# neale/safelife-k2

Measured on AMD Instinct MI355X. Metric: env-steps/sec (whole node) on 64×64 boards, batch 65536; bit-exact vs CPU ref, higher is better.
Workload: dtype u16; 1 GPU; 64x64 proc-gen prune-still, PPO wrapper chain; envs_per_gpu=65536, burnin_steps=400, global_batch=65536, parallelism=dp1 (env shards), obs=none, rng=philox, board_mode=auto, read_board=False

## Files before the change

### include/safelife_hip.h

```cpp
#ifndef SAFELIFE_HIP_H
#define SAFELIFE_HIP_H

#include <stdint.h>

#ifdef __cplusplus
extern "C" {
#endif

#define SL_OK 0
#define SL_EINVAL (-1)
#define SL_EHIP (-2)
#define SL_ETOOBIG (-3)

#define SL_RNG_STREAM 0
#define SL_RNG_PHILOX 1

#define SL_KERNEL_AUTO 0
#define SL_KERNEL_GENERIC 1
#define SL_KERNEL_FAST 2
#define SL_KERNEL_BANDS 3

#define SL_STREAM_ERR_RANGE 1
#define SL_STREAM_ERR_THRESHOLD 2

#define SL_BOARD_AUTO 0
#define SL_BOARD_UINT16 1

#define SL_MAX_EXITS 8
#define SL_BONUS_PERIOD_MAX 16

#define SL_OBS_NONE 0
#define SL_OBS_PACKED 1
#define SL_OBS_CHANNELS 2
#define SL_OBS_CHANNELS_U8 3
#define SL_OBS_CHANNELS_F32 4
#define SL_OBS_CHANNELS_BF16 5

const char *sl_version(void);
const char *sl_build_id(void);
int sl_device_arch(char *buf, int len);

int sl_event_create(void **ev);
int sl_event_destroy(void *ev);
int sl_event_elapsed_ms(void *begin, void *end, float *ms);
int sl_copy16(const void *src, void *dst, int64_t n16, void *stream);


int sl_advance(const uint16_t *in, uint16_t *out, int64_t B, int H, int W,
               const float *spawn_prob, float spawn_prob_scalar, int rng_mode,
               uint64_t seed, uint32_t env0, uint32_t step, uint32_t tensor,
               const double *draws, const int64_t *draw_offsets, void *stream);

int sl_count_eligible(const uint16_t *in, int64_t *counts, int64_t B, int H, int W,
                      void *stream);

int64_t sl_host_advance(const uint16_t *in, uint16_t *out, int64_t H, int64_t W,
                        float spawn_prob, const double *draws, int64_t n_draws);

int sl_exclusive_scan_i64(const int64_t *in, int64_t *out, int64_t n,
                          const int64_t *base, int64_t *total_out, void *stream);


#define SL_MT_PREFIX 21216
#define SL_MT_CTL_WORDS 8
#define SL_MT_POLY_WORDS 640
typedef struct sl_mt19937 {
    int32_t n_chains;
    int32_t rounds;
    int64_t ring_draws;
    double *ring;
    uint32_t *chains;
    uint32_t *prefix;
    uint32_t *polys;
    int64_t *ctl;
    void *ahead_stream;
    void *ev_fill, *ev_ahead;
    int32_t ahead_pending;
    int32_t bit_ring;
    double bits_thr;
} sl_mt19937;

int sl_mt19937_seed(sl_mt19937 *mt, uint32_t seed, int64_t first_draw, void *stream);
int sl_mt19937_fill(const sl_mt19937 *mt, const int64_t *lo, const int64_t *hi, int64_t *err,
                    void *stream);
int sl_mt19937_lookahead(sl_mt19937 *mt, void *ahead_stream);
int sl_mt19937_release(sl_mt19937 *mt);
int sl_mt19937_host_window(uint32_t seed, uint32_t *window624);
int sl_mt19937_host_jump_poly(uint64_t n, uint32_t *poly);
int sl_mt19937_host_jump(const uint32_t *window_in, const uint32_t *poly, uint32_t *window_out);
int sl_mt19937_host_draws(const uint32_t *window, int64_t n, double *out);


int sl_emd_cells(const double *p, const double *q, const int32_t *ys, const int32_t *xs,
                 int64_t n, const double *cost_table, int H, int W,
                 double extra_mass_penalty, double *out);

int sl_side_effect_workspace(int64_t E, int H, int W, int64_t *bytes);
int sl_side_effect_densities(const uint16_t *init_board, const uint16_t *final_board,
                             const int32_t *num_steps_dev, const int32_t *num_steps_host,
                             const float *spawn_prob, int64_t E, int H, int W,
                             int num_samples, int rng_mode, uint64_t seed, uint32_t env0,
                             const double *draws, int64_t *stream_pos, int max_keys,
                             uint16_t *keys, int32_t *n_keys, int32_t *present,
                             double *inaction, double *action, void *workspace,
                             int64_t workspace_bytes, void *stream);
int sl_side_effect_densities_k(const uint16_t *init_board, const uint16_t *final_board,
                               const int32_t *num_steps_dev, const int32_t *num_steps_host,
                               const float *spawn_prob, int64_t E, int H, int W,
                               int num_samples, int rng_mode, uint64_t seed, uint32_t env0,
// ... 181 lines not shown
```

### safelife-k2_amd/csrc/sl_bits.h

```cpp
#pragma once
#include "sl_action.h"


namespace sl {
namespace bits {

typedef uint32_t u32;

__device__ __forceinline__ u32 maj(u32 a, u32 b, u32 c) { return (a & b) | (c & (a | b)); }
__device__ __forceinline__ u32 mux(u32 s, u32 a, u32 b) { return (s & a) | (~s & b); }

template <int CTRL>
__device__ __forceinline__ u32 dpp(u32 v) {
    return (u32)__builtin_amdgcn_mov_dpp((int)v, CTRL, 0xF, 0xF, false);
}
__device__ __forceinline__ u32 lane_m1(u32 v) { return dpp<0x13C>(v); }
__device__ __forceinline__ u32 lane_p1(u32 v) { return dpp<0x134>(v); }
__device__ __forceinline__ u32 lane_x1(u32 v) { return dpp<0xB1>(v); }

struct H3 {
    u32 l0, r1;
};
struct V3 {
    u32 up, dn;
// ... 548 lines not shown
    __device__ int baseline() const { return rec(V, R_BASE); }
    __device__ int exit_count() const { return rec(V, R_EXC); }
    __device__ int exit_y(int e) const {
        return (int)(int16_t)(rec(V, R_EY + (e >> 1)) >> (16 * (e & 1)));
    }
    __device__ int exit_x(int e) const {
        return (int)(int16_t)(rec(V, R_EX + (e >> 1)) >> (16 * (e & 1)));
    }
    __device__ int game_over() const { return go; }
    __device__ int agent_x() const { return ax; }
    __device__ int agent_y() const { return ay; }
    __device__ int prior_len() const { return rec(V, R_PLEN); }
    __device__ int prior_head() const { return rec(V, R_PHEAD); }
    __device__ int prior_x(int k) const { return rec(V, R_PX + k); }
    __device__ int prior_y(int k) const { return rec(V, R_PY + k); }
    __device__ int side_effect() const { return rec(V, R_SIDE); }
    __device__ double bonus(int) const { return bval; }
};


__device__ __forceinline__ SpawnCtx spawn_ctx(const StepArgs &a, int64_t b, int spawn_bits) {
    SpawnCtx sc;
    sc.gid = a.env0 + (uint32_t)b;
    sc.step = a.step;
    sc.seed = a.seed;
    set_spawn_prob(sc, __int_as_float(spawn_bits));
    return sc;
}

template <int MODE>
__device__ __forceinline__ StreamSrc stream_src(const StepArgs &a, int64_t *scratch, int64_t B,
                                                int64_t b, int64_t &pos_b, int64_t &pos_g) {
    StreamSrc src{a.draws, a.n_draws, nullptr, a.draw_mask, a.draw_bits};
    pos_b = 0;
    pos_g = 0;
    if (MODE == SPAWN_STREAM) {
        const Scratch w = scratch_of(scratch, B);
        src.err = w.err;
        pos_b = w.offsets[2 * b];
        pos_g = w.offsets[2 * b + 1];
    }
    return src;
}

__device__ __forceinline__ RecFields rec_fields(const StepArgs &a, u32 V, int go, int ax, int ay) {
    RecFields fl{V, go, ax, ay, 0.0};
    if (a.bonus_period > 0)
        fl.bval = a.bonus_table[bonus_dist(fl.ax, fl.ay, fl.prior_x(fl.prior_head()),
                                           fl.prior_y(fl.prior_head()), fl.prior_len(),
                                           a.bonus_period, a.bonus_len)];
    return fl;
}

struct ScoreTotals {
    int points, score, possible, side;
};
__device__ __forceinline__ ScoreTotals score_totals(int pts, int scr, int pos, int side) {
    const int s1 = wave_total((pts + 192) | ((scr + 64) << 16));
    const int s2 = wave_total(pos | (side << 16));
    return ScoreTotals{(s1 & 0xFFFF) - 192 * 64, ((s1 >> 16) & 0xFFFF) - 64 * 64, s2 & 0xFFFF,
                       (s2 >> 16) & 0xFFFF};
}

struct Words2 {
    u32 w[2];
};
__device__ __forceinline__ Words2 recolour_exits(u32 P[32], bool can) {
    Words2 d9;
#pragma unroll
    for (int w = 0; w < 2; w++) {
        const u32 o9 = PL(P, 9, w);
        PL(P, 9, w) = can ? (o9 | PL(P, 8, w)) : (o9 & ~PL(P, 8, w));
        d9.w[w] = o9 ^ PL(P, 9, w);
    }
    return d9;
}

__device__ __forceinline__ void queue_reset(int64_t *scratch, int64_t B, uint32_t step, int64_t b) {
    int64_t *cnt = scratch + 8 * B + 2 + (step & 1);
    const int i = (int)atomicAdd((unsigned long long *)cnt, 1ull);
    reset_list(scratch)[i] = (int32_t)b;
}

}
}
```

### safelife-k2_amd/csrc/sl_bits.hip

```cpp
#include "sl_bits_geo.h"
#include "sl_obs.h"

using namespace sl;
using namespace sl::fast;
using namespace sl::bits;

namespace {

constexpr int kMinWaves = 4;
constexpr int kMinWavesObs = 3;

constexpr int N = 64;

typedef __attribute__((address_space(3))) u32 lds_u32;

__device__ __forceinline__ void dma_board(const uint16_t *__restrict__ src, lds_u32 *buf,
                                          int lane) {
    const char *s = reinterpret_cast<const char *>(src);
#pragma unroll
    for (int k = 0; k < 8; k++) {
        const int q = k * 64 + lane, row = q >> 3, pos = q & 7;
        const int c = (pos - ((row >> 5) << 2)) & 7;
        __builtin_amdgcn_global_load_lds((const void *)(s + row * 128 + c * 16),
                                         (__attribute__((address_space(3))) void *)(buf + k * 256),
// ... 656 lines not shown
struct PlaneSlots {
    static constexpr bool kFixed = K16 == kKeepC3;
    u32 keep;
    u32 store;
    __device__ __forceinline__ u32 keep32() const { return K16 ? K16 * 0x10001u : keep; }
    __device__ __forceinline__ u32 store32() const {
        return kFixed ? (K16 & ~kAgentC3) * 0x10001u : store;
    }
    __device__ __forceinline__ bool kept(int q) const { return (keep32() >> q) & 1u; }
    __device__ __forceinline__ bool stored(int q) const { return (store32() >> q) & 1u; }
    __device__ __forceinline__ u32 agent16() const {
        return kFixed ? kAgentC3 : (keep32() & ~store32()) & 0xFFFFu;
    }
    __device__ __forceinline__ int pos(int q) const {
        if (kFixed) return __builtin_popcount(store32() & ((1u << q) - 1u));
        u32 k = store;
        asm volatile("" : "+s"(k));
        return __builtin_popcount(k & ((1u << q) - 1u));
    }
    __device__ __forceinline__ int stored16() const { return __builtin_popcount(store32() & 0xFFFFu); }
    static __device__ __forceinline__ PlaneSlots of(u32 zero, u32 agent) {
        const u32 k = ~zero & 0xFFFFu;
        return PlaneSlots{k * 0x10001u, (k & ~agent) * 0x10001u};
    }
};
__device__ __forceinline__ void agent_words(int ay, int ax, int lane, u32 aw[2]) {
    const u32 bit = lane == 2 * (ax >> 1) + (ay >> 5) ? 1u << (ay & 31) : 0u;
    aw[0] = (ax & 1) ? 0u : bit;
    aw[1] = (ax & 1) ? bit : 0u;
}
constexpr int kMinWavesPlanes = 5;
constexpr int planes_min_waves(u32 k16, int obs) {
    return (obs == 0 && k16 == kKeepC3) ? kMinWavesPlanes : kMinWaves;
}

template <u32 K16>
__device__ __forceinline__ void dma_planes(const u32 *__restrict__ bp, PlaneSlots<K16> ps,
                                           lds_u32 *buf, int lane) {
    const int groups = (2 * ps.stored16() + 3) >> 2;
    const char *s = reinterpret_cast<const char *>(bp);
#pragma unroll
    for (int g = 0; g < 8; g++)
        if (g < groups)
            __builtin_amdgcn_global_load_lds((const void *)(s + g * 1024 + lane * 16),
                                             (__attribute__((address_space(3))) void *)(buf + g * 256),
                                             16, 0, 2);
}

__device__ __forceinline__ int near_cell_index(int k, int y0, int x0) {
    const int dy = k < 5 ? 0 : (k == 5 ? -1 : k == 6 ? 1 : k == 7 ? -2 : 2);
    const int dx = k >= 5 || k == 0 ? 0 : (k == 1 ? -1 : k == 2 ? 1 : k == 3 ? -2 : 2);
    return ((y0 + dy) & 63) * 64 + ((x0 + dx) & 63);
}
struct NearCells {
    int y0, x0;
    u32 v;
    __device__ __forceinline__ uint32_t operator()(int i) const {
        const int dy = (((i >> 6) - y0 + 32) & 63) - 32, dx = (((i & 63) - x0 + 32) & 63) - 32;
        const int k = dy == 0 ? (dx == 0 ? 0 : dx == -1 ? 1 : dx == 1 ? 2 : dx == -2 ? 3 : 4)
                              : (dy == -1 ? 5 : dy == 1 ? 6 : dy == -2 ? 7 : 8);
        return (u32)__builtin_amdgcn_readlane((int)v, __builtin_amdgcn_readfirstlane(k));
    }
};
template <u32 K16>
__device__ __forceinline__ u32 lds_plane_cell(const lds_u32 *buf, PlaneSlots<K16> ps, int i) {
    const int y = i >> 6, x = i & 63;
    const lds_u32 *q = buf + 2 * (x >> 1) + (y >> 5);
    const u32 r = (u32)(y & 31);
    const int w = 16 * (x & 1);
    u32 v = 0;
#pragma unroll
    for (int p = 0; p < 16; p++) {
        const int pw = ps.pos(p) + (w ? ps.stored16() : 0);
        if (ps.stored(p)) v |= ((q[pw * 64] >> r) & 1u) << p;
    }
    return v;
}

template <u32 K16, int OBS>
__global__ void __launch_bounds__(64, planes_min_waves(K16, OBS))
k_env_step_bits64_planes(StepKArgs ka) {
    __shared__ __attribute__((aligned(16))) u32 stage[N * N / 2];
    uint16_t *const vm = nullptr;
    constexpr bool GRAY = false, W6 = false;
#include "sl_planes64_step.inc"
}

template <u32 K16, int OBS>
__global__ void __launch_bounds__(64, planes_min_waves(K16, OBS))
k_env_planes64_gray(StepKArgs ka) {
    static_assert(OBS <= 1, "channel views load the three colour planes");
    __shared__ __attribute__((aligned(16))) u32 stage[N * N / 2];
    uint16_t *const vm = nullptr;
    constexpr bool GRAY = true, W6 = false;
#include "sl_planes64_step.inc"
}

constexpr int kMinWavesW6 = 6;
constexpr int kStageDwW6 = 1536;
template <u32 K16>
__global__ void __launch_bounds__(64, kMinWavesW6)
k_env_planes64_w6(StepKArgs ka) {
    __shared__ __attribute__((aligned(16))) u32 stage[kStageDwW6];
    uint16_t *const vm = nullptr;
    constexpr int OBS = 0;
    constexpr bool GRAY = true, W6 = true;
#include "sl_planes64_step.inc"
}

template <u32 K16, int ESZ>
__global__ void __launch_bounds__(64, kMinWaves)
k_env_planes64_chan(StepKArgs ka) {
    constexpr int OBS = ESZ == 1 ? 3 : (ESZ == 4 ? 4 : 2);
    __shared__ __attribute__((aligned(16))) u32 stage[N * N / 2];
    __shared__ __attribute__((aligned(16))) uint16_t vmask[sl::obs::kFusedChanCells];
    uint16_t *const vm = vmask;
    constexpr bool GRAY = false, W6 = false;
#include "sl_planes64_step.inc"
}

__global__ void __launch_bounds__(64) k_board_sync64(sl_env_state st, int demote) {
    const int64_t b = blockIdx.x;
    const int lane = threadIdx.x;
    const int pok = __builtin_amdgcn_readfirstlane(st.planes_ok[b]);
    if (!(pok & SL_POK_BOARD_PLANES)) return;
    if (!(pok & SL_POK_BOARD_FULL)) {
        const PlaneSlots<0> ps = PlaneSlots<0>::of(st.board_zero, st.agent_planes);
        const u32 *bp = st.planes + b * 4096 + lane;
        u32 P[32];
#pragma unroll
        for (int q = 0; q < 32; q++) P[q] = ps.stored(q) ? bp[ps.pos(q) * 64] : 0u;
        u32 aw[2];
        agent_words(__builtin_amdgcn_readfirstlane(st.agent_y[b]),
                    __builtin_amdgcn_readfirstlane(st.agent_x[b]), lane, aw);
#pragma unroll
        for (int q = 0; q < 32; q++)
            if ((ps.agent16() >> (q & 15)) & 1u) P[q] = aw[q >> 4];
        transpose32(P);
        u32 *gb = reinterpret_cast<u32 *>(st.board + b * (int64_t)(N * N)) + (lane & 1) * 1024 +
                  (lane >> 1);
#pragma unroll
        for (int y = 0; y < 32; y++) gb[y * 32] = P[y];
    }
    if (lane == 0)
        st.planes_ok[b] = demote ? pok & ~(SL_POK_BOARD_PLANES | SL_POK_BOARD_FULL)
                                 : pok | SL_POK_BOARD_FULL;
}

__global__ void __launch_bounds__(64)
k_stream_prologue64(StepKArgs ka) {
    const sl_env_state &st = ka.st;
    const int64_t b = blockIdx.x;
    const int lane = threadIdx.x;
    const int64_t off = b * (int64_t)(N * N);
    const int lane_off = (lane & 1) * 1024 + (lane >> 1);
    const u32 V = load_record(st, ka.actions, b, lane);
    const Scratch w = scratch_of(ka.fx.scratch, st.B);
    const int spf = rec(V, R_SPF) | (ka.ctp ? 1 : 0);
    SpawnCtx sc{0u, 0u, 0ull, 0.0};
    u32 P[32], ch[2];
    int nb = 0;
    if (spf & 1) {
        load_pairs_nt<32>(reinterpret_cast<const u32 *>(st.board + off) + lane_off, P);
        transpose32(P);
        Geo64<SPAWN_COUNT> gbd{lane, StreamSrc{nullptr, 0, nullptr}, 0, 0};
        rule_planes(P, ch, gbd, sc, 0u);
        nb = wave_total(gbd.count);
    }
    const int pok = (st.planes && st.planes_ok) ? rec(V, R_POK) & kPokGoalsSkip : 0;
    int ng = 0;
    if ((pok & kPokGoalsSkip) != kPokGoalsSkip && (spf & 2)) {
        if (pok & SL_POK_GOALS_MIRROR) {
            const u32 *mg = st.planes + b * 4096 + 2048 + lane;
#pragma unroll
            for (int q = 0; q < 32; q++) P[q] = mg[q * 64];
        } else {
            load_pairs_nt<32>(reinterpret_cast<const u32 *>(st.goals + off) + lane_off, P);
            transpose32(P);
        }
        Geo64<SPAWN_COUNT> ggl{lane, StreamSrc{nullptr, 0, nullptr}, 0, 0};
        rule_planes(P, ch, ggl, sc, 1u);
        ng = wave_total(ggl.count);
    }
    if (lane == 0) {
        w.counts[2 * b] = nb;
        w.counts[2 * b + 1] = ng;
    }
}

__global__ void __launch_bounds__(64)
k_env_reset_list(sl_env_state st, sl_level_pool pool, ResetArgs ra, int64_t *scratch,
                 uint32_t step, sl::obs::ObsArgs oa, uint64_t chpack, uint32_t one,
                 uint16_t *obs_out) {
    __shared__ __attribute__((aligned(16))) uint16_t vmask[sl::obs::kFusedChanCells];
    int64_t *cnt = scratch + 8 * st.B + 2;
    if (blockIdx.x == 0 && threadIdx.x == 0) cnt[(step + 1) & 1] = 0;
    const int32_t *list = reset_list(scratch);
    const int first = list[blockIdx.x];
    const int n = (int)__builtin_amdgcn_readfirstlane((int)cnt[step & 1]);
    for (int i = blockIdx.x; i < n; i += gridDim.x) {
        const int64_t b = __builtin_amdgcn_readfirstlane(i == (int)blockIdx.x ? first : list[i]);
        wave_reset(st, pool, ra, b, threadIdx.x);
        if (obs_out) {
            wait_vm();
            const sl::obs::ChanMap cm{chpack, oa.nch};
            uint8_t *o8 = reinterpret_cast<uint8_t *>(obs_out);
            if (oa.mode == SL_OBS_PACKED)
                sl::obs::obs_packed_wave(st, oa, b, threadIdx.x, obs_out);
            else if (oa.mode == SL_OBS_CHANNELS_U8)
                sl::obs::obs_channels_wave<1>(st, oa, cm, one, b, threadIdx.x, vmask, o8);
            else if (oa.mode == SL_OBS_CHANNELS_F32)
                sl::obs::obs_channels_wave<4>(st, oa, cm, one, b, threadIdx.x, vmask, o8);
            else
                sl::obs::obs_channels_wave<2>(st, oa, cm, one, b, threadIdx.x, vmask, o8);
        }
    }
}

int obs_kind(const FastExtra &fx) {
    if (!fx.obs_out) return 0;
    switch (fx.obs_mode) {
    case SL_OBS_PACKED: return 1;
    case SL_OBS_CHANNELS_U8: return 3;
    case SL_OBS_CHANNELS_F32: return 4;
    default: return 2;
    }
}

template <int MODE>
void launch_bits64(int kind, unsigned grid, const StepKArgs &ka, hipStream_t s) {
    switch (kind) {
    case 0: hipLaunchKernelGGL((k_env_step_bits64<0, MODE>), dim3(grid), dim3(64), 0, s, ka); break;
    case 1: hipLaunchKernelGGL((k_env_step_bits64<1, MODE>), dim3(grid), dim3(64), 0, s, ka); break;
    case 2: hipLaunchKernelGGL((k_env_step_bits64<2, MODE>), dim3(grid), dim3(64), 0, s, ka); break;
    case 3: hipLaunchKernelGGL((k_env_step_bits64<3, MODE>), dim3(grid), dim3(64), 0, s, ka); break;
    default: hipLaunchKernelGGL((k_env_step_bits64<4, MODE>), dim3(grid), dim3(64), 0, s, ka); break;
    }
}

template <u32 K16>
void launch_planes64_chan_k(int esz, unsigned grid, const StepKArgs &ka, hipStream_t s) {
    switch (esz) {
    case 1: hipLaunchKernelGGL((k_env_planes64_chan<K16, 1>), dim3(grid), dim3(64), 0, s, ka); break;
    case 4: hipLaunchKernelGGL((k_env_planes64_chan<K16, 4>), dim3(grid), dim3(64), 0, s, ka); break;
    default: hipLaunchKernelGGL((k_env_planes64_chan<K16, 2>), dim3(grid), dim3(64), 0, s, ka); break;
    }
}

void launch_planes64_chan(u32 keep, int esz, unsigned grid, const StepKArgs &ka, hipStream_t s) {
    if (keep == kKeepC3Fixed) launch_planes64_chan_k<kKeepC3>(esz, grid, ka, s);
    else if (keep == kKeepAll) launch_planes64_chan_k<kKeepAll>(esz, grid, ka, s);
    else launch_planes64_chan_k<0>(esz, grid, ka, s);
}

}

namespace sl {

bool planes64_shape(const sl_env_state &st) {
    return st.H == N && st.W == N && st.planes && st.planes_ok && st.board_planes == st.planes;
}

int sync_board_planes64(const sl_env_state &st, int demote, hipStream_t s) {
    if (!planes64_shape(st) || st.B <= 0) return SL_OK;
    hipLaunchKernelGGL(k_board_sync64, dim3((unsigned)st.B), dim3(64), 0, s, st, demote);
    return hipGetLastError() == hipSuccess ? SL_OK : SL_EHIP;
}

int launch_step_bits(const sl_env_state &st, const StepArgs &a, const FastExtra &fx,
                     const int32_t *actions, int ctp, int ctc, double *reward, uint8_t *done,
                     uint8_t *flags, int32_t *ep_len, int32_t *ep_rew, hipStream_t s,
                     int planes64_waves) {
    if (st.H != N || st.W != N) return SL_ETOOBIG;
    const unsigned grid = (unsigned)st.B;
    const StepKArgs ka{st, a, fx, actions, ctp, ctc, reward, done, flags, ep_len, ep_rew};
    if (fx.obs_out && (fx.obs_vh < 1 || fx.obs_vw < 1 || fx.obs_vh * fx.obs_vw > 4096))
        return SL_EINVAL;
    if (fx.stream) {
        if (stream_counts(fx)) {
            const int rca = launch_env_action(st, actions, ctp, ctc, scratch_of(fx.scratch, st.B).act, s);
            if (rca) return rca;
            hipLaunchKernelGGL(k_stream_prologue64, dim3(grid), dim3(64), 0, s, ka);
            if (hipGetLastError() != hipSuccess) return SL_EHIP;
        }
        const int rc = stream_offsets(st, fx, s);
        if (rc || !stream_steps(fx)) return rc;
        if (fx.ev_begin) (void)hipEventRecord((hipEvent_t)fx.ev_begin, s);
        launch_bits64<SPAWN_STREAM>(obs_kind(fx), grid, ka, s);
    } else {
        if (fx.ev_begin) (void)hipEventRecord((hipEvent_t)fx.ev_begin, s);
        if (fx.plane_mode) {
            u32 keep = ~st.board_zero & 0xFFFFu;
            if (keep == kKeepC3) keep = st.agent_planes == kAgentC3 ? kKeepC3Fixed : 0u;
            const int kind = obs_kind(fx);
            if (kind >= 2) {
                launch_planes64_chan(keep, obs_esz(kind), grid, ka, s);
            } else if (keep == kKeepC3Fixed && st.goals_gray) {
                if (kind)
                    hipLaunchKernelGGL((k_env_planes64_gray<kKeepC3, 1>), dim3(grid), dim3(64), 0, s, ka);
                else if (planes64_waves == 5)
                    hipLaunchKernelGGL((k_env_planes64_gray<kKeepC3, 0>), dim3(grid), dim3(64), 0, s, ka);
                else
                    hipLaunchKernelGGL((k_env_planes64_w6<kKeepC3>), dim3(grid), dim3(64), 0, s, ka);
            } else if (fx.obs_out) {
                if (keep == kKeepC3Fixed)
                    hipLaunchKernelGGL((k_env_step_bits64_planes<kKeepC3, 1>), dim3(grid), dim3(64), 0, s, ka);
                else if (keep == kKeepAll)
                    hipLaunchKernelGGL((k_env_step_bits64_planes<kKeepAll, 1>), dim3(grid), dim3(64), 0, s, ka);
                else
                    hipLaunchKernelGGL((k_env_step_bits64_planes<0, 1>), dim3(grid), dim3(64), 0, s, ka);
            } else if (keep == kKeepC3Fixed) {
                hipLaunchKernelGGL((k_env_step_bits64_planes<kKeepC3, 0>), dim3(grid), dim3(64), 0, s, ka);
            } else if (keep == kKeepAll) {
                hipLaunchKernelGGL((k_env_step_bits64_planes<kKeepAll, 0>), dim3(grid), dim3(64), 0, s, ka);
            } else {
                hipLaunchKernelGGL((k_env_step_bits64_planes<0, 0>), dim3(grid), dim3(64), 0, s, ka);
            }
        }
        else
            launch_bits64<SPAWN_PHILOX>(obs_kind(fx), grid, ka, s);
    }
    if (hipGetLastError() != hipSuccess) return SL_EHIP;
    if (fx.ev_end) (void)hipEventRecord((hipEvent_t)fx.ev_end, s);
    if (fx.capture) {
        const int rc = launch_capture(st, *fx.capture, flags, 0, s);
        if (rc) return rc;
    }
    if (fx.fuse_reset && fx.pool.K > 0) {
        const unsigned grid = (unsigned)(st.B < 512 ? st.B : 512);
        sl::obs::ObsArgs oa{};
        oa.vh = fx.obs_vh;
        oa.vw = fx.obs_vw;
        oa.remove_white = fx.obs_rw;
        oa.mode = fx.obs_mode;
        oa.nch = fx.obs_nch;
        hipLaunchKernelGGL(k_env_reset_list, dim3(grid), dim3(64), 0, s, st, fx.pool, fx.ra,
                           fx.scratch, a.step, oa, fx.obs_chpack, fx.obs_one, fx.obs_out);
    }
    return hipGetLastError() == hipSuccess ? SL_OK : SL_EHIP;
}

}
```

### safelife-k2_amd/csrc/sl_env.hip

```cpp
#include "sl_env_common.h"
#include "sl_env_action.h"
#include "sl_obs.h"

#include <math.h>

using namespace sl;
using namespace sl::obs;

namespace {

constexpr int NT = 256;
constexpr int kMaxCells = 16384;

template <bool DELTAS>
__global__ void __launch_bounds__(256)
k_env_action(sl_env_state st, const int32_t *__restrict__ actions, int ctp, int ctc,
             int64_t *__restrict__ act) {
    const int64_t b = (int64_t)blockIdx.x * blockDim.x + threadIdx.x;
    if (b >= st.B) return;
    env_action_one<DELTAS>(st, actions, ctp, ctc, act, b);
}

__device__ __forceinline__ void stage(uint16_t *dst, const uint16_t *src, int hw) {
    if ((((uintptr_t)src) & 15) == 0 && (hw & 7) == 0) {
// ... 847 lines not shown
    if (!rc) st->planes_live = 0;
    return rc;
}

static void draws_from_ring(StepArgs &a, const sl_mt19937 &mt) {
    a.draws = mt.ring;
    a.n_draws = INT64_MAX;
    a.draw_mask = mt.ring_draws - 1;
    if (mt.bit_ring) {
        a.draw_bits = reinterpret_cast<const uint32_t *>(mt.ring);
        a.bits_thr = mt.bits_thr;
    }
}

extern "C" int sl_env_step(sl_env_state *st, const sl_level_pool *pool, const int32_t *actions,
                           const sl_env_cfg *cfg, double *reward, uint8_t *done,
                           uint8_t *info_flags, int32_t *ep_len, int32_t *ep_reward,
                           void *stream) {
    if (!state_ok(st) || !cfg || !actions || !reward || !done || !cfg->scratch) return SL_EINVAL;
    if (cfg->bonus_period < 0 || cfg->bonus_period > SL_BONUS_PERIOD_MAX) return SL_EINVAL;
    if (cfg->bonus_period > 0 && (!cfg->bonus_table || cfg->bonus_len < 1)) return SL_EINVAL;
    if (cfg->auto_reset && (!pool || !info_flags || pool->K <= 0 || pool->H != st->H ||
                            pool->W != st->W))
        return SL_EINVAL;
    const int64_t B = st->B;
    if (B == 0) return SL_OK;
    hipStream_t s = (hipStream_t)stream;
    Scratch sc = scratch_of(cfg->scratch, B);
    const size_t lds = (size_t)2 * st->H * st->W * sizeof(uint16_t);

    StepArgs a;
    a.time_limit = cfg->time_limit;
    a.auto_reset = cfg->auto_reset;
    a.bonus_len = cfg->bonus_len;
    a.bonus_period = cfg->bonus_period;
    a.penalty_coef = cfg->penalty_coef;
    a.bonus_table = cfg->bonus_table;
    a.seed = cfg->seed;
    a.step = cfg->step;
    a.env0 = cfg->env0;
    a.draws = cfg->draws;
    a.n_draws = cfg->n_draws;

    if (cfg->rng_mode != SL_RNG_STREAM && cfg->rng_mode != SL_RNG_PHILOX) return SL_EINVAL;
    const bool replay = cfg->rng_mode == SL_RNG_STREAM;
    if (replay && cfg->mt) draws_from_ring(a, *cfg->mt);
    if (replay && (!cfg->stream_pos || (!a.draws && a.n_draws > 0))) return SL_EINVAL;
    if (cfg->stream_phase < 0 || cfg->stream_phase > 2 || (cfg->stream_phase && !replay) ||
        (cfg->stream_phase == 2 && !cfg->stream_base))
        return SL_EINVAL;
    if (cfg->kernel == SL_KERNEL_BANDS) return SL_EINVAL;
    const bool bits_ok = cfg->kernel != SL_KERNEL_GENERIC;
    const bool fast = bits_ok && st->H == 64 && st->W == 64;
    const bool fast128 = bits_ok && bits128_shape(*st);
    const bool small = bits_ok && !fast && small_shape(*st);
    if (cfg->kernel == SL_KERNEL_FAST && !fast && !fast128 && !small) return SL_ETOOBIG;
    bool reset_done = false;
    FastExtra fx;
    fx.fuse_reset = cfg->auto_reset ? 1 : 0;
    if (pool) fx.pool = *pool;
    else fx.pool = sl_level_pool{};
    fx.ra = reset_args(cfg);
    fx.scratch = cfg->scratch;
    fx.ev_end = cfg->ev_end;
    const sl_capture *cap = (cfg->capture && cfg->capture->n > 0) ? cfg->capture : nullptr;
    if (cap && (!cap->env || !cap->flags || !info_flags || !cfg->auto_reset)) return SL_EINVAL;
    fx.capture = cap;
    fx.stream = replay ? 1 : 0;
    fx.stream_pos = cfg->stream_pos;
    fx.stream_phase = cfg->stream_phase;
    fx.stream_base = cfg->stream_base;
    fx.mt = replay ? cfg->mt : nullptr;
    if (fx.mt && fx.mt->bit_ring) fx.bits_thr = fx.mt->bits_thr;
    fx.ev_begin = cfg->ev_begin;
    if (cap && small) fx.fuse_reset = 0;
    ObsArgs oa;
    if (cfg->obs_out) {
        const int rc = obs_args(cfg->obs_vh, cfg->obs_vw, cfg->obs_remove_white, cfg->obs_mode,
                                cfg->obs_channels, cfg->obs_nch, &oa);
        if (rc) return rc;
    }
    const bool planes128 = st->board_planes && st->planes_ok && st->H == 128 && st->W == 128;
    if (cfg->board_mode != SL_BOARD_AUTO && cfg->board_mode != SL_BOARD_UINT16) return SL_EINVAL;
    if (cfg->planes64_waves != 0 && cfg->planes64_waves != 5 && cfg->planes64_waves != 6)
        return SL_EINVAL;
    const bool fuse_obs128 = fast128 && planes128 && cfg->obs_out && !cap &&
                             cfg->board_mode != SL_BOARD_UINT16 &&
                             (!replay || st->elig_planes) && oa.mode == SL_OBS_PACKED &&
                             oa.vh <= kViewMaxRows128 && oa.vw <= 128;
    fx.plane_mode = (fast128 && planes128 && (!cfg->obs_out || fuse_obs128) && !cap &&
                     (!replay || st->elig_planes) && cfg->board_mode != SL_BOARD_UINT16) ? 1 : 0;
    const bool fuse_obs =
        cfg->obs_out && fast &&
        ((oa.mode == SL_OBS_PACKED && oa.vh * oa.vw <= kObsMaxCells) ||
         (oa.mode != SL_OBS_PACKED && oa.vh <= 64 && oa.vw <= 64 &&
          oa.vh * oa.vw + 2 <= kFusedChanCells && (((uintptr_t)cfg->obs_out) & 15) == 0));
    const bool planes64 = planes64_shape(*st);
    if (planes64)
        fx.plane_mode = (fast && !cap && !replay && cfg->board_mode != SL_BOARD_UINT16 &&
                         (!cfg->obs_out || fuse_obs)) ? 1 : 0;
    if ((planes128 || planes64) && !fx.plane_mode) {
        const int rc = demote_planes(st, s);
        if (rc) return rc;
    }
    if (fx.plane_mode && cfg->stream_phase != 1) st->planes_live = 1;
    fx.obs_out = (fuse_obs || fuse_obs128) ? (uint16_t *)cfg->obs_out : nullptr;
    fx.obs_vh = cfg->obs_vh;
    fx.obs_vw = cfg->obs_vw;
    fx.obs_rw = cfg->obs_remove_white;
    fx.obs_mode = SL_OBS_PACKED;
    fx.obs_nch = 0;
    fx.obs_chpack = 0;
    fx.obs_one = 1u;
    if (cfg->obs_out) {
        fx.obs_mode = oa.mode;
        fx.obs_nch = oa.nch;
        for (int k = 0; k < oa.nch; k++) fx.obs_chpack |= (uint64_t)oa.ch[k] << (4 * k);
        fx.obs_one = oa.mode == SL_OBS_CHANNELS_F32 ? 0x3F800000u
                     : oa.mode == SL_OBS_CHANNELS_BF16 ? 0x3F80u : 1u;
    }
    if (fast128) {
        int rc = launch_step_bits128(*st, a, fx, actions, cfg->can_toggle_powers,
                                     cfg->can_toggle_colors, reward, done, info_flags, ep_len,
                                     ep_reward, s);
        if (rc || cfg->stream_phase == 1) return rc;
        reset_done = fx.fuse_reset && fx.pool.K > 0;
    } else if (small) {
        int rc = launch_step_small(*st, a, fx, actions, cfg->can_toggle_powers,
                                   cfg->can_toggle_colors, reward, done, info_flags, ep_len,
                                   ep_reward, s);
        if (rc || cfg->stream_phase == 1) return rc;
        reset_done = fx.fuse_reset && fx.pool.K > 0 && fx.pool.H == st->H && fx.pool.W == st->W;
    } else if (fast) {
        int rc = launch_step_bits(*st, a, fx, actions, cfg->can_toggle_powers,
                                  cfg->can_toggle_colors, reward, done, info_flags, ep_len,
                                  ep_reward, s, cfg->planes64_waves);
        if (rc || cfg->stream_phase == 1) return rc;
        reset_done = fx.fuse_reset && fx.pool.K > 0;
    } else {
        if (!replay || stream_counts(fx)) {
            hipLaunchKernelGGL(k_env_action<true>, dim3((unsigned)((B + 255) / 256)), dim3(256), 0,
                               s, *st, actions, cfg->can_toggle_powers, cfg->can_toggle_colors,
                               sc.act);
            if (hipGetLastError() != hipSuccess) return SL_EHIP;
        }
        if (replay) {
            if (stream_counts(fx)) {
                if (!set_lds((const void *)k_env_count, lds)) return SL_ETOOBIG;
                hipLaunchKernelGGL(k_env_count, dim3((unsigned)B), dim3(NT), lds, s, *st, sc.counts);
                if (hipGetLastError() != hipSuccess) return SL_EHIP;
            }
            int rc = stream_offsets(*st, fx, s);
            if (rc || cfg->stream_phase == 1) return rc;
            if (!set_lds((const void *)k_env_step_generic<SL_RNG_STREAM>, lds)) return SL_ETOOBIG;
            hipLaunchKernelGGL(k_env_step_generic<SL_RNG_STREAM>, dim3((unsigned)B), dim3(NT), lds,
                               s, *st, a, sc.act, sc.offsets, sc.err, reward, done, info_flags,
                               ep_len, ep_reward);
        } else {
            if (!set_lds((const void *)k_env_step_generic<SL_RNG_PHILOX>, lds)) return SL_ETOOBIG;
            if (cfg->ev_begin) (void)hipEventRecord((hipEvent_t)cfg->ev_begin, s);
            hipLaunchKernelGGL(k_env_step_generic<SL_RNG_PHILOX>, dim3((unsigned)B), dim3(NT), lds,
                               s, *st, a, sc.act, sc.offsets, sc.err, reward, done, info_flags,
                               ep_len, ep_reward);
        }
    }
    if (hipGetLastError() != hipSuccess) return SL_EHIP;
    if (cfg->ev_end && !fast && !fast128) (void)hipEventRecord((hipEvent_t)cfg->ev_end, s);
// ... 163 lines not shown
```

### safelife-k2_amd/csrc/sl_planes64_step.inc

```
    const sl_env_state &st = ka.st;
    const StepArgs &a = ka.a;
    const FastExtra &fx = ka.fx;
    const int64_t b = blockIdx.x;
    const int lane = threadIdx.x;
    lds_u32 *buf = (lds_u32 *)&stage[0];
    const PlaneSlots<K16> ps = PlaneSlots<K16>::of(st.board_zero, st.agent_planes);
    constexpr int kStageDw = (int)(sizeof(stage) / sizeof(u32));
    static_assert(!W6 || (PlaneSlots<K16>::kFixed && OBS == 0), "W6: fixed planes, no views");
    static_assert(!W6 || 2 * __builtin_popcount(K16 & ~kAgentC3 & 0xFFFFu) * 64 <= kStageDw,
                  "the stored plane words fit the buffer");
    static_assert(pool_rows_dwords(K16 ? K16 : 0xFFFFu, W6) <= kStageDw,
                  "the pool's start-plane rows fit the buffer");
    static_assert(kStageDw >= (W6 ? N * N / 4 : N * N / 2), "a board, or half of one (W6)");
    Pre pre;
    const bool gray_blank = GRAY && (!OBS || fx.obs_rw != 0);
    if (!GRAY) issue_pre(st, ka.actions, b, lane, pre);
    else if (gray_blank) issue_pre<0>(st, ka.actions, b, lane, pre);
    else issue_pre<1>(st, ka.actions, b, lane, pre);
    dma_planes(st.planes + b * 4096, ps, buf, lane);
    const int64_t off = b * (int64_t)(N * N);
    const int lane_off = (lane & 1) * 1024 + (lane >> 1);
    u32 *gg = reinterpret_cast<u32 *>(st.goals + off) + lane_off;
    u32 *mg = st.planes + b * 4096 + 2048 + lane;
    u32 *bp = st.planes + b * 4096 + lane;
// ... 109 lines not shown
    int pts, scr, pos, side;
    const u32 gblack[3][2] = {{0u, 0u}, {0u, 0u}, {0u, 0u}};
    if (W6 && roll >= 0) {
        const int dy = roll >> 16, dx = roll & 0xFFFF;
        int p1, s1, o1, e1;
        pool_planes_lds_word<KEEP, 0>(buf, dy, dx, lane, PS);
        score_planes<false, 0, 1>(PB, GRAY ? gblack : gcol, PS, &pts, &scr, &pos, &side);
        __builtin_amdgcn_sched_barrier(0);
        pool_planes_lds_word<KEEP, 1>(buf, dy, dx, lane, PS);
        score_planes<false, 1, 2>(PB, GRAY ? gblack : gcol, PS, &p1, &s1, &o1, &e1);
        pts += p1;
        scr += s1;
        pos += o1;
        side += e1;
    } else
    score_planes(PB, GRAY ? gblack : gcol, PS, &pts, &scr, &pos, &side);
    const ScoreTotals tot = score_totals(pts, scr, pos, side);
    __builtin_amdgcn_sched_barrier(0);

    const Words2 d9 = recolour_exits(
        PB, can_exit_now(fl.min_performance(), tot.score, fl.baseline(), tot.possible));
    u32 em[2] = {0u, 0u};
#pragma unroll
    for (int k = 0; k < 4; k++) {
        if (k < ne) {
            const int y = eidx[k] >> 6, x = eidx[k] & 63;
            const u32 bit = lane == 2 * (x >> 1) + (y >> 5) ? 1u << (y & 31) : 0u;
            em[x & 1] |= bit;
        }
    }
    u32 dw[2], dall[2];
#pragma unroll
    for (int w = 0; w < 2; w++) {
        dw[w] = cb[w] | em[w];
        dall[w] = em[w] | (((held_lanes >> lane) & 1ull) ? cb[w] : 0u);
    }
    if (!pin || wave_or(dw[0] | dw[1] | d9.w[0] | d9.w[1])) {
#pragma unroll
        for (int k = 0; k < 16; k++) {
            if (!ps.stored(k)) continue;
#pragma unroll
            for (int w = 0; w < 2; w++) {
                const u32 d = (k == 0 || k == 3 || k == 10 || k == 11) ? dw[w]
                              : k == 9 ? (dw[w] | d9.w[w]) : dall[w];
                if (!pin || d)
                    __builtin_nontemporal_store(PL(PB, k, w), &bp[ps.pos(k + 16 * w) * 64]);
            }
        }
    }
    const int ok = gok | SL_POK_BOARD_PLANES;
    if (ok != pok_all && lane == 0) st.planes_ok[b] = ok;
    if (OBS) {
        const bool rw = kernarg().fx.obs_rw != 0;
#pragma unroll
        for (int w = 0; w < 2; w++) {
            if (GRAY && rw) continue;
            u32 g0 = gcol[0][w], g1 = gcol[GRAY ? 0 : 1][w], g2 = gcol[GRAY ? 0 : 2][w];
            if (rw) {
                const u32 wh = g0 & g1 & g2;
                g0 &= ~wh;
                g1 &= ~wh;
                g2 &= ~wh;
            }
            const u32 b12 = PL(PB, 12, w), b13 = PL(PB, 13, w), b14 = PL(PB, 14, w);
            u32 c = b12 & g0;
            PL(PB, 12, w) = b12 ^ g0;
            const u32 x13 = b13 ^ g1;
            PL(PB, 13, w) = x13 ^ c;
            c = (b13 & g1) | (c & x13);
            const u32 x14 = b14 ^ g2;
            PL(PB, 14, w) = x14 ^ c;
            c = (b14 & g2) | (c & x14);
            PL(PB, 15, w) ^= c;
        }
        transpose32(PB);
        lds_put_board(buf, lane, PB);
        __builtin_amdgcn_fence(__ATOMIC_SEQ_CST, "wavefront");
        __builtin_amdgcn_wave_barrier();
        __builtin_amdgcn_sched_barrier(0);
        if (OBS >= 2) write_obs_channels<obs_esz(OBS)>(buf, vm, fl, b, lane);
        else write_obs(buf, fx, fl, b, lane);
        __builtin_amdgcn_sched_barrier(0);
    }
    int reset = 0;
    if (lane == 0)
        reset = epilogue_core(st, a, b, fl, act_reward, tot.points, tot.score, tot.possible,
                              tot.side, ka.reward_out, ka.done_out, ka.flags_out, ka.ep_len_out,
                              ka.ep_rew_out);
    reset = __builtin_amdgcn_readfirstlane(reset);
    if (fx.fuse_reset && reset && lane == 0) queue_reset(fx.scratch, st.B, a.step, b);
```

### safelife-k2_amd/safelife_amd/_lib.py

```python
import ctypes
import os
import subprocess

_HERE = os.path.dirname(os.path.abspath(__file__))
_DEFAULT_LIB = os.path.join(_HERE, "_native", "libsafelife_hip.so")
LIB_PATH = os.environ.get("SAFELIFE_HIP_LIB") or _DEFAULT_LIB
CSRC = os.path.join(os.path.dirname(_HERE), "csrc")

SL_OK, SL_EINVAL, SL_EHIP, SL_ETOOBIG = 0, -1, -2, -3
SL_RNG_STREAM, SL_RNG_PHILOX = 0, 1
SL_KERNEL_AUTO, SL_KERNEL_GENERIC, SL_KERNEL_FAST = 0, 1, 2
SL_KERNEL_BANDS = 3
SL_STREAM_ERR_RANGE, SL_STREAM_ERR_THRESHOLD = 1, 2
SL_EMD_DEVICE_MAX_CELLS = 256
SL_EMD_ST_BADCELL, SL_EMD_ST_TOOBIG, SL_EMD_ST_PIVOTS = -1, -2, -3
SL_BOARD_AUTO, SL_BOARD_UINT16 = 0, 1
SL_MAX_EXITS = 8
SL_BONUS_PERIOD_MAX = 16
SL_OBS_NONE, SL_OBS_PACKED, SL_OBS_CHANNELS, SL_OBS_CHANNELS_U8 = 0, 1, 2, 3
SL_OBS_CHANNELS_F32, SL_OBS_CHANNELS_BF16 = 4, 5
SL_POK_GOALS_MIRROR, SL_POK_GOALS_FIXED, SL_POK_ELIG, SL_POK_GOALS_SIX = 2, 4, 8, 16
SL_POK_GOALS_LEVEL, SL_POK_BOARD_PLANES, SL_POK_BOARD_FULL, SL_POK_BOARD_LO12 = 32, 64, 128, 256
SL_POK_GOALS = SL_POK_GOALS_MIRROR | SL_POK_GOALS_FIXED | SL_POK_GOALS_SIX | SL_POK_GOALS_LEVEL
SL_POK_BOARD = SL_POK_BOARD_PLANES | SL_POK_BOARD_FULL | SL_POK_BOARD_LO12

_ERRORS = {SL_EINVAL: "invalid argument / shape", SL_EHIP: "HIP launch error",
           SL_ETOOBIG: "board too large for this kernel"}

vp = ctypes.c_void_p
i32 = ctypes.c_int32
i64 = ctypes.c_int64
u32 = ctypes.c_uint32
u64 = ctypes.c_uint64
f32 = ctypes.c_float
f64 = ctypes.c_double


class EnvState(ctypes.Structure):
    _fields_ = [("B", i64), ("H", i32), ("W", i32),
                ("board", vp), ("goals", vp), ("start_board", vp),
                ("agent_x", vp), ("agent_y", vp), ("orientation", vp),
                ("game_over", vp), ("episode_length", vp), ("episode_reward", vp),
                ("old_points", vp), ("baseline", vp), ("score", vp), ("possible", vp),
                ("side_effect", vp), ("spawn_prob", vp), ("min_performance", vp),
                ("prior_x", vp), ("prior_y", vp), ("prior_len", vp), ("prior_head", vp),
                ("exit_count", vp), ("exit_y", vp), ("exit_x", vp),
                ("level_index", vp), ("episodes", vp), ("num_steps", vp),
                ("spawn_flags", vp), ("start_roll", vp), ("planes", vp), ("planes_ok", vp),
                ("elig_planes", vp), ("board_planes", vp), ("board_zero", u32),
                ("planes_live", i32), ("agent_planes", u32), ("goals_gray", u32)]


class LevelPool(ctypes.Structure):
    _fields_ = [("K", i32), ("H", i32), ("W", i32),
                ("board", vp), ("goals", vp), ("agent_x", vp), ("agent_y", vp),
                ("orientation", vp), ("spawn_prob", vp), ("min_performance", vp),
                ("board_planes", vp), ("goal_planes", vp)]


class EnvCfg(ctypes.Structure):
    _fields_ = [("time_limit", i32), ("auto_reset", i32),
                ("can_toggle_powers", i32), ("can_toggle_colors", i32),
                ("penalty_coef", f64), ("wrapper_min_performance", f64),
                ("bonus_table", vp), ("bonus_len", i32), ("bonus_period", i32),
                ("rng_mode", i32), ("seed", u64), ("step", u32), ("env0", u32),
                ("draws", vp), ("n_draws", i64), ("stream_pos", vp), ("scratch", vp),
                ("level_mode", i32), ("n_total_envs", i32), ("augment_roll", i32),
                ("ev_begin", vp), ("ev_end", vp), ("kernel", i32),
                ("obs_out", vp), ("obs_mode", i32), ("obs_vh", i32), ("obs_vw", i32),
                ("obs_remove_white", i32), ("obs_nch", i32), ("obs_channels", i32 * 16),
                ("capture", vp), ("stream_phase", i32), ("stream_base", vp), ("mt", vp),
                ("board_mode", i32), ("planes64_waves", i32)]


class MT19937(ctypes.Structure):
    _fields_ = [("n_chains", i32), ("rounds", i32), ("ring_draws", i64), ("ring", vp),
                ("chains", vp), ("prefix", vp), ("polys", vp), ("ctl", vp),
                ("ahead_stream", vp), ("ev_fill", vp), ("ev_ahead", vp),
                ("ahead_pending", i32), ("bit_ring", i32), ("bits_thr", f64)]


class Capture(ctypes.Structure):
    _fields_ = [("n", i32), ("env", vp), ("board", vp), ("goals", vp), ("orientation", vp),
                ("flags", vp), ("reset_board", vp), ("reset_goals", vp),
                ("reset_orientation", vp),
                ("start_board", vp), ("score", vp), ("possible", vp), ("baseline", vp),
                ("num_steps", vp), ("spawn_prob", vp), ("min_performance", vp),
                ("episode_length", vp), ("episode_reward", vp), ("level_index", vp)]


_lib = None


class HipUnavailable(RuntimeError):
    pass


def build(force=False):
    if force or not os.path.exists(LIB_PATH):
# ... 121 lines not shown
```

### safelife-k2_amd/safelife_amd/vec_env.py

```python
import ctypes
import math

import numpy as np

from . import _lib
from .levels import LevelPool
from .spaces import Box, env_spaces

ACTION_NAMES = ("NULL", "MOVE UP", "MOVE RIGHT", "MOVE DOWN", "MOVE LEFT",
                "TOGGLE UP", "TOGGLE RIGHT", "TOGGLE DOWN", "TOGGLE LEFT")


class GlobalCounter:

    def __init__(self):
        self.episodes_started = 0
        self.episodes_completed = 0
        self.num_steps = 0


def _sched(val, counter):
    return val(counter.num_steps) if callable(val) else val


# ... 9 lines not shown
AGENT_PLANE_BITS = 0x0062


def agent_planes(board, agent_x, agent_y, can_toggle_powers=False):
    board = np.asarray(board, dtype=np.uint16)
    K = board.shape[0]
    if K == 0:
        return 0
    cand = AGENT_PLANE_BITS & ~(0x00E1 if can_toggle_powers else 0)
    at = board[np.arange(K), np.asarray(agent_y), np.asarray(agent_x)]
    if not (at & 0x0010).all():
        return 0
    mask = 0
    for k in range(16):
        bit = 1 << k
        if not cand & bit:
            continue
        n = ((board & bit) != 0).reshape(K, -1).sum(1)
        if (n == 1).all() and ((at & bit) != 0).all():
            mask |= bit
    return mask


def goals_gray(goals):
    g = np.asarray(goals, dtype=np.uint16)
    r, gr, b = (g >> 9) & 1, (g >> 10) & 1, (g >> 11) & 1
    return int(bool(((r == gr) & (r == b)).all()))


def start_board_hi_bits(start_board):
    import torch
    return ((start_board.view(torch.int16) & 0x7000) != 0).flatten(1).any(1)


class SafeLifeVecEnv:
    action_names = ACTION_NAMES

    def __init__(self, levels, num_envs, device=None, *, time_limit=1000,
                 view_shape=(15, 15), output_channels=tuple(range(15)),
                 remove_white_goals=True, movement_bonus=0.1, movement_bonus_power=0.01,
                 movement_bonus_period=4, penalty_coef=0.0, min_performance=0.01,
                 auto_reset=True, rng="philox", seed=0, spawn_stream=None,
                 level_order="sequential", augment_roll=False, env0=0, n_total_envs=None,
                 can_toggle_powers=False, can_toggle_colors=False, obs_dtype="uint16",
                 compute_obs=True, global_counter=None, kernel="auto", stream_exchange=None,
                 stream_ring="auto", board_mode="auto", planes64_waves=6):
        import torch
        self.torch = torch
        self.device = _lib.require_device(device)
        self.pool = levels if isinstance(levels, LevelPool) else LevelPool.from_levels(levels)
        self.B = int(num_envs)
        self.H, self.W = self.pool.H, self.pool.W
        self.time_limit = int(time_limit)
        self.view_shape = tuple(int(v) for v in view_shape)
        self.output_channels = tuple(output_channels) if output_channels else None
        self.remove_white_goals = bool(remove_white_goals)
        self.movement_bonus = movement_bonus
        self.movement_bonus_power = movement_bonus_power
        self.movement_bonus_period = int(movement_bonus_period)
        if not 0 <= self.movement_bonus_period <= _lib.SL_BONUS_PERIOD_MAX:
            raise ValueError("movement_bonus_period must be in [0, %d]" % _lib.SL_BONUS_PERIOD_MAX)
        self.penalty_coef = penalty_coef
        self.min_performance = min_performance
        self.auto_reset = bool(auto_reset)
        self.rng = rng
        self.seed = int(seed)
        self.level_order = level_order
        self.augment_roll = bool(augment_roll)
        self.env0 = int(env0)
        self.n_total_envs = int(n_total_envs) if n_total_envs else self.B
        self.can_toggle_powers = bool(can_toggle_powers)
        self.can_toggle_colors = bool(can_toggle_colors)
        self.compute_obs = bool(compute_obs)
        self.kernel = {"auto": _lib.SL_KERNEL_AUTO, "generic": _lib.SL_KERNEL_GENERIC,
                       "fast": _lib.SL_KERNEL_FAST}[kernel]
        self.global_counter = global_counter if global_counter is not None else GlobalCounter()
        self.stream_exchange = stream_exchange
        if stream_ring not in ("auto", "doubles"):
            raise ValueError("stream_ring must be 'auto' or 'doubles'")
        self.stream_ring = stream_ring
        if board_mode not in ("auto", "planes", "uint16"):
            raise ValueError("board_mode must be 'auto', 'planes' or 'uint16'")
        self.board_mode = board_mode
        if planes64_waves not in (5, 6):
            raise ValueError("planes64_waves must be 5 or 6")
        self.planes64_waves = planes64_waves
        self._board_read_at = None
        self._step_index = 0
        self._last_step = None
        self._abandoned = 0
        self._synced = (0, 0)
        self._recorder = None
        self._draw_base = 0
        self._last_mode = None
        self._alloc(obs_dtype)
        self._may_spawn = self.pool.has_spawners()
        self.action_space, self.observation_space = env_spaces(
            ACTION_NAMES, self.view_shape, self.output_channels)
        if self.output_channels is not None and obs_dtype != "uint16":
            self.observation_space = Box(0, 1, self.observation_space.shape,
                                         np.uint8 if obs_dtype == "uint8" else np.float32)
        self.mt = None
        if rng == "stream":
            if spawn_stream is None:
                self.spawn_stream = None
                self.mt = self._make_mt(0, self._pool_threshold(self.pool)
                                        if stream_ring == "auto" else None)
            else:
                self.set_spawn_stream(spawn_stream)
        elif rng != "philox":
            raise ValueError("rng must be 'philox' or 'stream'")
        self._bonus_key = None

    def _alloc(self, obs_dtype):
        torch, dev, B, H, W = self.torch, self.device, self.B, self.H, self.W
        z = lambda *s, dt=torch.int32: torch.zeros(s, dtype=dt, device=dev)
        self._board = z(B, H, W, dt=torch.uint16)
        self.goals = z(B, H, W, dt=torch.uint16)
        self.start_board = z(B, H, W, dt=torch.uint16)
        self.st_t = {
            "agent_x": z(B), "agent_y": z(B), "orientation": z(B), "game_over": z(B),
            "episode_length": z(B), "episode_reward": z(B), "old_points": z(B),
            "baseline": z(B), "score": z(B), "possible": z(B), "side_effect": z(B),
            "spawn_prob": z(B, dt=torch.float32), "min_performance": z(B, dt=torch.float64),
            "prior_x": z(B, _lib.SL_BONUS_PERIOD_MAX), "prior_y": z(B, _lib.SL_BONUS_PERIOD_MAX),
            "prior_len": z(B), "prior_head": z(B), "exit_count": z(B),
            "exit_y": z(B, _lib.SL_MAX_EXITS, dt=torch.int16),
            "exit_x": z(B, _lib.SL_MAX_EXITS, dt=torch.int16),
            "level_index": z(B), "episodes": z(B), "num_steps": z(B), "spawn_flags": z(B),
            "start_roll": z(B) - 1,
        }
        s = _lib.EnvState()
        s.B, s.H, s.W = B, H, W
        s.board, s.goals, s.start_board = (self._board.data_ptr(), self.goals.data_ptr(),
                                           self.start_board.data_ptr())
        for k, t in self.st_t.items():
            setattr(s, k, t.data_ptr())
        self.planes_ok = z(B)
        if (H, W) in ((64, 64), (128, 128)):
            self.planes = z(B, H // 32, 32, 64)
            s.planes = self.planes.data_ptr()
            s.planes_ok = self.planes_ok.data_ptr()
        self.board_planes = None
        if (H, W) == (64, 64):
            self.board_planes = self.planes
            s.board_planes = self.planes.data_ptr()
            s.board_zero = self._zero_planes(self._pool_bits(self.pool))
            s.agent_planes = self._agent_planes(self.pool)
            s.goals_gray = goals_gray(self.pool.goals)
        if (H, W) == (128, 128):
            self.board_planes = z(B, H // 32, 32, 64)
            s.board_planes = self.board_planes.data_ptr()
            s.board_zero = self._zero_planes(self._pool_bits(self.pool))
        if (H, W) == (128, 128) and self.rng == "stream":
            self.elig_planes = z(B, 1024)
            s.elig_planes = self.elig_planes.data_ptr()
        self._state = s
        self.actions_dev = z(B)
        self.reward = z(B, dt=torch.float64)
        self.done = z(B, dt=torch.uint8)
        self.flags = z(B, dt=torch.uint8)
        self.ep_len = z(B)
        self.ep_rew = z(B)
        self.scratch = z(8 * B + 16, dt=torch.int64)
        self.stream_pos = z(1, dt=torch.int64)
        vh, vw = self.view_shape
        if self.output_channels is None:
            self.obs_mode = _lib.SL_OBS_PACKED
# ... 569 lines not shown
```

Before: 582.5 million env-steps/s.

## Split 64x64 W6 step epilogue and reset into a separate tail kernel

```diff
diff --git a/include/safelife_hip.h b/include/safelife_hip.h
--- a/include/safelife_hip.h
+++ b/include/safelife_hip.h
@@ -25,6 +25,8 @@
 
 #define SL_BOARD_AUTO 0
 #define SL_BOARD_UINT16 1
+
+#define SL_PLANES64_W6_UNSPLIT (-6)
 
 #define SL_MAX_EXITS 8
 #define SL_BONUS_PERIOD_MAX 16
diff --git a/safelife-k2_amd/csrc/sl_bits.h b/safelife-k2_amd/csrc/sl_bits.h
--- a/safelife-k2_amd/csrc/sl_bits.h
+++ b/safelife-k2_amd/csrc/sl_bits.h
@@ -654,5 +654,29 @@
     reset_list(scratch)[i] = (int32_t)b;
 }
 
-}
-}
+struct Handover {
+    int act_reward, points, score, possible, side;
+    int go, ax, ay;
+};
+typedef int i32x4 __attribute__((ext_vector_type(4)));
+__device__ __forceinline__ i32x4 *handover_of(int64_t *scratch, int64_t B) {
+    return reinterpret_cast<i32x4 *>(scratch + 4 * B);
+}
+__device__ __forceinline__ void put_handover(i32x4 *hv, int64_t b, const Handover &h) {
+    hv[2 * b] = i32x4{h.act_reward, h.points, h.score, h.possible};
+    hv[2 * b + 1] = i32x4{h.side, h.go, h.ax, h.ay};
+}
+__device__ __forceinline__ Handover get_handover(const i32x4 *hv, int64_t b) {
+    const i32x4 u = hv[2 * b], v = hv[2 * b + 1];
+    return Handover{u.x, u.y, u.z, u.w, v.x, v.y, v.z, v.w};
+}
+
+struct HandFields : GlobalFields {
+    int go, ax, ay;
+    __device__ int game_over() const { return go; }
+    __device__ int agent_x() const { return ax; }
+    __device__ int agent_y() const { return ay; }
+};
+
+}
+}
diff --git a/safelife-k2_amd/csrc/sl_bits.hip b/safelife-k2_amd/csrc/sl_bits.hip
--- a/safelife-k2_amd/csrc/sl_bits.hip
+++ b/safelife-k2_amd/csrc/sl_bits.hip
@@ -762,7 +762,7 @@
 k_env_step_bits64_planes(StepKArgs ka) {
     __shared__ __attribute__((aligned(16))) u32 stage[N * N / 2];
     uint16_t *const vm = nullptr;
-    constexpr bool GRAY = false, W6 = false;
+    constexpr bool GRAY = false, W6 = false, SPLIT_EPI = false;
 #include "sl_planes64_step.inc"
 }
 
@@ -772,7 +772,7 @@
     static_assert(OBS <= 1, "channel views load the three colour planes");
     __shared__ __attribute__((aligned(16))) u32 stage[N * N / 2];
     uint16_t *const vm = nullptr;
-    constexpr bool GRAY = true, W6 = false;
+    constexpr bool GRAY = true, W6 = false, SPLIT_EPI = false;
 #include "sl_planes64_step.inc"
 }
 
@@ -784,8 +784,54 @@
     __shared__ __attribute__((aligned(16))) u32 stage[kStageDwW6];
     uint16_t *const vm = nullptr;
     constexpr int OBS = 0;
-    constexpr bool GRAY = true, W6 = true;
+    constexpr bool GRAY = true, W6 = true, SPLIT_EPI = false;
 #include "sl_planes64_step.inc"
+}
+
+template <u32 K16>
+__global__ void __launch_bounds__(64, kMinWavesW6)
+k_env_planes64_s6(StepKArgs ka) {
+    __shared__ __attribute__((aligned(16))) u32 stage[kStageDwW6];
+    uint16_t *const vm = nullptr;
+    constexpr int OBS = 0;
+    constexpr bool GRAY = true, W6 = true, SPLIT_EPI = true;
+#include "sl_planes64_step.inc"
+}
+
+constexpr int kTailThreads = 256;
+__global__ void __launch_bounds__(kTailThreads)
+k_env_epilogue_reset64(sl_env_state st, StepArgs a, sl_level_pool pool, ResetArgs ra,
+                       int64_t *scratch, double *reward_out, uint8_t *done_out,
+                       uint8_t *flags_out, int32_t *ep_len_out, int32_t *ep_rew_out) {
+    const int64_t b = (int64_t)blockIdx.x * kTailThreads + threadIdx.x;
+    const int lane = threadIdx.x & 63;
+    if (b == 0) scratch[8 * st.B + 2 + ((a.step + 1) & 1)] = 0;
+    bool reset = false;
+    if (b < st.B) {
+        const Handover h = get_handover(handover_of(scratch, st.B), b);
+        const HandFields f{{st, b, a.bonus_table}, h.go, h.ax, h.ay};
+        reset = epilogue_core(st, a, b, f, h.act_reward, h.points, h.score, h.possible, h.side,
+                              reward_out, done_out, flags_out, ep_len_out, ep_rew_out);
+    }
+    __shared__ uint64_t finished[kTailThreads / 64];
+    const int wave = __builtin_amdgcn_readfirstlane((int)(threadIdx.x >> 6));
+    const uint64_t mine = __ballot(reset);
+    if (lane == 0) finished[wave] = mine;
+    __builtin_amdgcn_fence(__ATOMIC_RELEASE, "workgroup");
+    __syncthreads();
+    const int64_t b0 = (int64_t)blockIdx.x * kTailThreads;
+    int i = 0;
+#pragma unroll 1
+    for (int q = 0; q < kTailThreads / 64; q++) {
+        const uint64_t f = finished[q];
+        uint64_t todo = ((uint64_t)(u32)__builtin_amdgcn_readfirstlane((int)(f >> 32)) << 32) |
+                        (u32)__builtin_amdgcn_readfirstlane((int)f);
+        while (todo) {
+            const int k = __builtin_ctzll(todo);
+            todo &= todo - 1;
+            if ((i++ & (kTailThreads / 64 - 1)) == wave) wave_reset(st, pool, ra, b0 + 64 * q + k, lane);
+        }
+    }
 }
 
 template <u32 K16, int ESZ>
@@ -795,7 +841,7 @@
     __shared__ __attribute__((aligned(16))) u32 stage[N * N / 2];
     __shared__ __attribute__((aligned(16))) uint16_t vmask[sl::obs::kFusedChanCells];
     uint16_t *const vm = vmask;
-    constexpr bool GRAY = false, W6 = false;
+    constexpr bool GRAY = false, W6 = false, SPLIT_EPI = false;
 #include "sl_planes64_step.inc"
 }
 
@@ -954,6 +1000,7 @@
     if (st.H != N || st.W != N) return SL_ETOOBIG;
     const unsigned grid = (unsigned)st.B;
     const StepKArgs ka{st, a, fx, actions, ctp, ctc, reward, done, flags, ep_len, ep_rew};
+    bool split = false;
     if (fx.obs_out && (fx.obs_vh < 1 || fx.obs_vw < 1 || fx.obs_vh * fx.obs_vw > 4096))
         return SL_EINVAL;
     if (fx.stream) {
@@ -973,6 +1020,9 @@
             u32 keep = ~st.board_zero & 0xFFFFu;
             if (keep == kKeepC3) keep = st.agent_planes == kAgentC3 ? kKeepC3Fixed : 0u;
             const int kind = obs_kind(fx);
+            split = keep == kKeepC3Fixed && st.goals_gray && kind == 0 && planes64_waves != 5 &&
+                    planes64_waves != SL_PLANES64_W6_UNSPLIT && fx.fuse_reset && fx.pool.K > 0 &&
+                    !fx.capture && fx.scratch && (reinterpret_cast<uintptr_t>(fx.scratch) & 15) == 0;
             if (kind >= 2) {
                 launch_planes64_chan(keep, obs_esz(kind), grid, ka, s);
             } else if (keep == kKeepC3Fixed && st.goals_gray) {
@@ -980,6 +1030,8 @@
                     hipLaunchKernelGGL((k_env_planes64_gray<kKeepC3, 1>), dim3(grid), dim3(64), 0, s, ka);
                 else if (planes64_waves == 5)
                     hipLaunchKernelGGL((k_env_planes64_gray<kKeepC3, 0>), dim3(grid), dim3(64), 0, s, ka);
+                else if (split)
+                    hipLaunchKernelGGL((k_env_planes64_s6<kKeepC3>), dim3(grid), dim3(64), 0, s, ka);
                 else
                     hipLaunchKernelGGL((k_env_planes64_w6<kKeepC3>), dim3(grid), dim3(64), 0, s, ka);
             } else if (fx.obs_out) {
@@ -1006,7 +1058,11 @@
         const int rc = launch_capture(st, *fx.capture, flags, 0, s);
         if (rc) return rc;
     }
-    if (fx.fuse_reset && fx.pool.K > 0) {
+    if (split) {
+        const unsigned tgrid = (unsigned)((st.B + kTailThreads - 1) / kTailThreads);
+        hipLaunchKernelGGL(k_env_epilogue_reset64, dim3(tgrid), dim3(kTailThreads), 0, s, st, a,
+                           fx.pool, fx.ra, fx.scratch, reward, done, flags, ep_len, ep_rew);
+    } else if (fx.fuse_reset && fx.pool.K > 0) {
         const unsigned grid = (unsigned)(st.B < 512 ? st.B : 512);
         sl::obs::ObsArgs oa{};
         oa.vh = fx.obs_vh;
diff --git a/safelife-k2_amd/csrc/sl_env.hip b/safelife-k2_amd/csrc/sl_env.hip
--- a/safelife-k2_amd/csrc/sl_env.hip
+++ b/safelife-k2_amd/csrc/sl_env.hip
@@ -953,7 +953,8 @@
     }
     const bool planes128 = st->board_planes && st->planes_ok && st->H == 128 && st->W == 128;
     if (cfg->board_mode != SL_BOARD_AUTO && cfg->board_mode != SL_BOARD_UINT16) return SL_EINVAL;
-    if (cfg->planes64_waves != 0 && cfg->planes64_waves != 5 && cfg->planes64_waves != 6)
+    if (cfg->planes64_waves != 0 && cfg->planes64_waves != 5 && cfg->planes64_waves != 6 &&
+        cfg->planes64_waves != SL_PLANES64_W6_UNSPLIT)
         return SL_EINVAL;
     const bool fuse_obs128 = fast128 && planes128 && cfg->obs_out && !cap &&
                              cfg->board_mode != SL_BOARD_UINT16 &&
diff --git a/safelife-k2_amd/csrc/sl_planes64_step.inc b/safelife-k2_amd/csrc/sl_planes64_step.inc
--- a/safelife-k2_amd/csrc/sl_planes64_step.inc
+++ b/safelife-k2_amd/csrc/sl_planes64_step.inc
@@ -215,6 +215,12 @@
         else write_obs(buf, fx, fl, b, lane);
         __builtin_amdgcn_sched_barrier(0);
     }
+    if (SPLIT_EPI) {
+        if (lane == 0)
+            put_handover(handover_of(fx.scratch, st.B), b,
+                         Handover{act_reward, tot.points, tot.score, tot.possible, tot.side,
+                                  fl.go, fl.ax, fl.ay});
+    } else {
     int reset = 0;
     if (lane == 0)
         reset = epilogue_core(st, a, b, fl, act_reward, tot.points, tot.score, tot.possible,
@@ -222,3 +228,4 @@
                               ka.ep_rew_out);
     reset = __builtin_amdgcn_readfirstlane(reset);
     if (fx.fuse_reset && reset && lane == 0) queue_reset(fx.scratch, st.B, a.step, b);
+    }
diff --git a/safelife-k2_amd/safelife_amd/_lib.py b/safelife-k2_amd/safelife_amd/_lib.py
--- a/safelife-k2_amd/safelife_amd/_lib.py
+++ b/safelife-k2_amd/safelife_amd/_lib.py
@@ -15,6 +15,7 @@
 SL_EMD_DEVICE_MAX_CELLS = 256
 SL_EMD_ST_BADCELL, SL_EMD_ST_TOOBIG, SL_EMD_ST_PIVOTS = -1, -2, -3
 SL_BOARD_AUTO, SL_BOARD_UINT16 = 0, 1
+SL_PLANES64_W6_UNSPLIT = -6
 SL_MAX_EXITS = 8
 SL_BONUS_PERIOD_MAX = 16
 SL_OBS_NONE, SL_OBS_PACKED, SL_OBS_CHANNELS, SL_OBS_CHANNELS_U8 = 0, 1, 2, 3
diff --git a/safelife-k2_amd/safelife_amd/vec_env.py b/safelife-k2_amd/safelife_amd/vec_env.py
--- a/safelife-k2_amd/safelife_amd/vec_env.py
+++ b/safelife-k2_amd/safelife_amd/vec_env.py
@@ -115,8 +115,8 @@
         if board_mode not in ("auto", "planes", "uint16"):
             raise ValueError("board_mode must be 'auto', 'planes' or 'uint16'")
         self.board_mode = board_mode
-        if planes64_waves not in (5, 6):
-            raise ValueError("planes64_waves must be 5 or 6")
+        if planes64_waves not in (5, 6, _lib.SL_PLANES64_W6_UNSPLIT):
+            raise ValueError("planes64_waves must be 5, 6 or -6")
         self.planes64_waves = planes64_waves
         self._board_read_at = None
         self._step_index = 0
```

Result: faster. 618.6 million env-steps/s (median of 6 runs) (+6.2%).
